# unirestore/UniRestore

Hardware: AMD Instinct MI355X
Metric: restored 512x512 images/sec @ 20 denoise steps (whole job) (higher is better)
Workload: dtype bf16; 1 GPU; PIR 512x512 batch=8/GPU, 20 DDIM steps, bf16, hipGraph replay (BASELINE.json configs[1]; configs[2] shape for N=8); global_batch=8, per_gpu_batch=8, image=512, denoise_steps=20, parallelism=image-parallel dp1, weights=seeded random init (no checkpoints reachable)

## Files before the change

### include/unirestore_hip.h

```cpp
#ifndef UNIRESTORE_HIP_H
#define UNIRESTORE_HIP_H

#include <stddef.h>
#include <stdint.h>

#ifdef __cplusplus
extern "C" {
#endif

typedef void* ur_stream_t;

enum { UR_OK = 0, UR_E_INVALID = -1, UR_E_UNSUPPORTED = -2, UR_E_LAUNCH = -3, UR_E_WORKSPACE = -4 };

enum { UR_DT_BF16 = 0, UR_DT_F16 = 1 };

enum {
  UR_ACT_NONE = 0,
  UR_ACT_SILU = 1,
  UR_ACT_GELU = 2,
  UR_ACT_GEGLU = 3,
  UR_ACT_GATE = 4,
  UR_ACT_TANH = 5,
  UR_ACT_RELU = 6
};
// ... 60 lines not shown
int ur_conv2d_plan_launch(const ur_conv_desc* d, ur_conv_launch_info* info);
int ur_conv_launcher_count(void);
const char* ur_conv_launcher_name(int i);

int ur_gemm_bias_act(const void* x, const void* w, const float* bias, const void* residual, void* y, long long M, int N, int K,
                     int ldx, int ldw, int ldy, int ldr, int act, float* workspace, size_t workspace_bytes, int dtype,
                     ur_stream_t stream);
int ur_groupconv3x3_nhwc(const void* x, const void* w, const float* bias, void* y, int N, int H, int W, int Cg, int Cog,
                         int groups, int act, float* workspace, size_t workspace_bytes, int dtype, ur_stream_t stream);

int ur_groupnorm_stats_parts(int N, int HW, int C);
size_t ur_groupnorm_ws_bytes(int N, int HW, int C);
size_t ur_groupnorm_ab_bytes(int N, int C);
int ur_groupnorm_stats(const void* x, float* part, int N, int HW, int C, int dtype, ur_stream_t stream);
int ur_instnorm_stats(const void* x, float* part, int N, int HW, int C, int dtype, ur_stream_t stream);
int ur_groupnorm_finalize(const float* part1, int parts1, int C1, const float* part2, int parts2, int C2, const float* gamma,
                          const float* beta, int N, int HW, int G, float eps, float* ab, float* mean_out, ur_stream_t stream);
int ur_groupnorm_apply_act(const void* x, const void* x2, void* y, const float* ab, int N, int HW, int C1, int C2, int silu,
                           int dtype, ur_stream_t stream);
int ur_groupnorm_nhwc(const void* x, const void* x2, void* y, const float* gamma, const float* beta, int N, int HW,
                      int C1, int C2, int G, float eps, int silu, float* ws, float* ab, const float* pre1, int parts1,
                      const float* pre2, int parts2, int dtype, ur_stream_t stream);
int ur_layernorm_rows(const void* x, void* y, const float* gamma, const float* beta, long long rows, int C,
                      float eps, int dtype, ur_stream_t stream);
int ur_softmax_rows_f32(const float* s, void* p, long long rows, int cols, int ldp, int dtype, ur_stream_t stream);

int ur_attention_fwd(const void* q, const void* k, const void* vt, void* o, int B, int H, int Tq, int Tk,
                     int D, int ldq, int ldk, int ldvt, int ldo, long long bs_q, long long bs_k,
                     long long bs_vt, long long bs_o, float scale, int dtype, ur_stream_t stream);
size_t ur_attention_workspace_bytes(int B, int H, int Tq, int Tk, int D);
// ... 81 lines not shown
```

### unirestore_amd/capi.py

```python
import ctypes as C
import os

import torch

_HERE = os.path.dirname(os.path.abspath(__file__))
LIB_PATH = os.environ.get("UR_LIB") or os.path.join(_HERE, "libunirestore_hip.so")

UR_ACT_NONE, UR_ACT_SILU, UR_ACT_GELU, UR_ACT_GEGLU, UR_ACT_GATE, UR_ACT_TANH, UR_ACT_RELU = range(7)
UR_DT_BF16, UR_DT_F16 = 0, 1
UR_E_INVALID, UR_E_UNSUPPORTED = -1, -2


class ConvDesc(C.Structure):
    _fields_ = [
        ("x", C.c_void_p), ("x2", C.c_void_p), ("w", C.c_void_p), ("bias", C.c_void_p), ("residual", C.c_void_p),
        ("y", C.c_void_p), ("yt", C.c_void_p), ("gn_part", C.c_void_p), ("gn_ab", C.c_void_p), ("gn_silu", C.c_int),
        ("row_stats", C.c_void_p), ("ln_stats", C.c_void_p), ("ln_colsum", C.c_void_p), ("ln_eps", C.c_float), ("ln_dim", C.c_int), ("ln_parts", C.c_int),
        ("workspace", C.c_void_p),
        ("workspace_bytes", C.c_size_t),
        ("N", C.c_int), ("H", C.c_int), ("W", C.c_int),
        ("C1", C.c_int), ("ldx", C.c_int), ("C2", C.c_int), ("ldx2", C.c_int),
        ("Cout", C.c_int), ("ldw", C.c_int), ("ldy", C.c_int), ("ldr", C.c_int),
        ("KH", C.c_int), ("KW", C.c_int), ("stride", C.c_int), ("pad_t", C.c_int), ("pad_l", C.c_int),
        ("OH", C.c_int), ("OW", C.c_int),
# ... 25 lines not shown
SIGNATURES = {
    "ur_version": (_I, []),
    "ur_last_error": (C.c_char_p, []),
    "ur_conv2d_nhwc": (_I, [C.POINTER(ConvDesc), _P]),
    "ur_conv2d_plan": (_I, [C.POINTER(ConvDesc), C.POINTER(ConvPlan)]),
    "ur_conv2d_plan_launch": (_I, [C.POINTER(ConvDesc), C.POINTER(ConvLaunchInfo)]),
    "ur_conv_launcher_count": (_I, []),
    "ur_conv_launcher_name": (C.c_char_p, [_I]),
    "ur_gemm_bias_act": (_I, [_P, _P, _P, _P, _P, _LL, _I, _I, _I, _I, _I, _I, _I, _P, _SZ, _I, _P]),
    "ur_groupconv3x3_nhwc": (_I, [_P, _P, _P, _P, _I, _I, _I, _I, _I, _I, _I, _P, _SZ, _I, _P]),
    "ur_groupnorm_stats_parts": (_I, [_I, _I, _I]),
    "ur_groupnorm_ws_bytes": (_SZ, [_I, _I, _I]),
    "ur_groupnorm_ab_bytes": (_SZ, [_I, _I]),
    "ur_groupnorm_stats": (_I, [_P, _P, _I, _I, _I, _I, _P]),
    "ur_instnorm_stats": (_I, [_P, _P, _I, _I, _I, _I, _P]),
    "ur_groupnorm_finalize": (_I, [_P, _I, _I, _P, _I, _I, _P, _P, _I, _I, _I, _F, _P, _P, _P]),
    "ur_groupnorm_apply_act": (_I, [_P, _P, _P, _P, _I, _I, _I, _I, _I, _I, _P]),
    "ur_groupnorm_nhwc": (_I, [_P, _P, _P, _P, _P, _I, _I, _I, _I, _I, _F, _I, _P, _P, _P, _I, _P, _I, _I, _P]),
    "ur_layernorm_rows": (_I, [_P, _P, _P, _P, _LL, _I, _F, _I, _P]),
    "ur_softmax_rows_f32": (_I, [_P, _P, _LL, _I, _I, _I, _P]),
    "ur_attention_fwd": (_I, [_P, _P, _P, _P, _I, _I, _I, _I, _I, _I, _I, _I, _I, _LL, _LL, _LL, _LL, _F, _I, _P]),
    "ur_attention_workspace_bytes": (_SZ, [_I, _I, _I, _I, _I]),
    "ur_attention_fwd_ws": (_I, [_P, _P, _P, _P, _I, _I, _I, _I, _I, _I, _I, _I, _I, _LL, _LL, _LL, _LL, _F, _P, _SZ, _I, _P]),
    "ur_attention_plan_launch": (_I, [_P, _P, _P, _P, _I, _I, _I, _I, _I, _I, _I, _I, _I, _LL, _LL, _LL, _LL, _P, _SZ, C.POINTER(AttentionPlan)]),
    "ur_attention_kernel_count": (_I, []),
    "ur_attention_kernel_name": (C.c_char_p, [_I]),
    "ur_chain_tile_bytes": (_SZ, []),
    "ur_ff_geglu_fused": (_I, [_P, _P, _SZ, _P, _LL, _I, _I, _I, _I, _F, _I, _P]),
    "ur_transformer_head_fused": (_I, [_P, _P, _P, _SZ, _P, _P, _P, _P, _LL, _I, _I, _F, _I, _P]),
    "ur_transformer_tail_fused": (_I, [_P, _P, _P, _P, _SZ, _P, _P, _LL, _I, _I, _I, _I, _I, _F, _F, _I, _P]),
# ... 79 lines not shown
```

### unirestore_amd/csrc/igemm.hip

```cpp
#include "igemm_impl.h"

namespace urk {
#define UR_DECLARE(name)                                                                                             \
  ConvLaunch name##_bf16(void* k, size_t ws_bytes);                                                                 \
  ConvLaunch name##_f16(void* k, size_t ws_bytes);                                                                  \
  static ConvLaunch name(ConvK& k, size_t ws_bytes) { return (k.f16 ? name##_f16 : name##_bf16)(&k, ws_bytes); }
UR_CONV_LAUNCHERS(UR_DECLARE)
#undef UR_DECLARE
}

namespace {

ConvLaunch dispatch_conv(ConvK& k, bool pair, size_t ws_bytes) {
  if (k.KH == 3 && k.stride == 1 && k.pad_t == 1 && k.pad_l == 1 && k.kcm && k.staged_ok_ && !pair && k.nbatch == 1 &&
      k.OW % 32 == 0 && k.OH % 8 == 0 && k.OH == (k.ups ? 2 * k.H : k.H) && k.OW == (k.ups ? 2 * k.W : k.W) && !k.yt) {
    const bool ok128 = k.Cout % 128 == 0, ok160 = k.Cout % 160 == 0;
    const long long tm8 = (long long)k.N * (k.OH / 8) * (k.OW / 32);
    auto eff = [](long long t) { return t <= 128 ? (double)(t * (256 / t)) / 256.0 : (double)t / (double)(((t + 255) / 256) * 256); };
    const bool use160 = ok160 && (!ok128 || eff(tm8 * (k.Cout / 160)) >= eff(tm8 * (k.Cout / 128)));
    const long long tiles8 = tm8 * (use160 ? k.Cout / 160 : k.Cout / 128);
    if ((ok128 || ok160) && tiles8 >= 64) {
      if (use160) return urk::halo_8x32_160(k, ws_bytes);
      return urk::halo_8x32_128(k, ws_bytes);
    }
// ... 12 lines not shown
    if (k.OH == 8 && k.OW == 8 && k.N % 4 == 0) {
      return urk::himg_8x8x4(k, ws_bytes);
    }
  }
  if (k.KH == 1 && k.stride == 1 && !k.ups && k.C2 == 0 && k.staged_ok_ && k.Cout % 256 == 0 && !k.yt && (k.act == UR_ACT_GEGLU || k.act == UR_ACT_GATE) &&
      (long long)((k.M + 255) / 256) * (k.Cout / 256) * k.nbatch >= 200 && (long long)k.M * k.ldx < (1ll << 31) - 256)
  {
    auto fill = [](long long t) { return (double)t / (double)(((t + 255) / 256) * 256); };
    const long long tm = (k.M + 255) / 256;
    if (k.Cout % 320 == 0 && k.nbatch == 1 && !k.bias_img && fill(tm * (k.Cout / 320)) > fill(tm * (k.Cout / 256)))
      return urk::gemm_256x320_pair(k, ws_bytes);
    return urk::gemm_256x256(k, ws_bytes);
  }
  const bool use_v1 = k.KH == 1 && k.nk <= 10;
  const long long blocks128 = (long long)((k.M + 127) / 128) * ((k.Cout + 127) / 128) * k.nbatch;
  const bool g1 = k.KH == 1 && k.stride == 1 && !k.ups && k.C2 == 0 && k.pad_t == 0 && k.pad_l == 0 && k.OH == k.H && k.OW == k.W &&
                  (long long)k.M * k.ldx + k.Ktot < (1ll << 31) - 256;
  auto nosplit = [&](int bm, int bn) { return (long long)((k.M + bm - 1) / bm) * ((k.Cout + bn - 1) / bn) * k.nbatch >= 200 || k.nk < 8 || !k.ws; };
  if (k.KH == 1 && !pair && k.Cout > 64) {
    const long long blocks64 = (long long)((k.M + 63) / 64) * ((k.Cout + 63) / 64) * k.nbatch;
    if (blocks128 < 200 && g1 && blocks64 >= 128 && blocks64 <= 256 && k.nk >= 8 && k.nk <= 48) return urk::g1_64x64_deep(k, ws_bytes);
    if (g1 && blocks128 < 200 && k.nk > 24 && k.nk <= 96 && (long long)((k.M + 127) / 128) * ((k.Cout + 63) / 64) * k.nbatch >= 256)
      return urk::g1_128x64_deep(k, ws_bytes);
    if (blocks128 < 200 && g1 && ((blocks64 >= 128 && k.nk <= 24) || (blocks64 >= 256 && k.nk <= 48))) return urk::g1_64x64(k, ws_bytes);
    if (blocks128 < 200 && k.nk <= 24) return g1 && nosplit(64, 64) ? urk::g1_64x64(k, ws_bytes) : urk::v1_64x64(k, ws_bytes);
    if (use_v1 && blocks128 > 256 && blocks128 < 400 && k.Cout % 128 == 0) return g1 && nosplit(128, 64) ? urk::g1_128x64(k, ws_bytes) : urk::v1_128x64(k, ws_bytes);
  }
  if (use_v1) {
    if (pair) return urk::v1_128x128(k, ws_bytes);
    if (k.Cout <= 32) return urk::v1_256x32(k, ws_bytes);
    if (k.Cout <= 64) return urk::v1_128x64(k, ws_bytes);
// ... 177 lines not shown
```

### unirestore_amd/csrc/igemm_g1.hip

```cpp
#include "igemm_impl.h"

#ifndef UR_NST_128x128
#define UR_NST_128x128 2
#endif
#ifndef UR_NST_128x160
#define UR_NST_128x160 2
#endif
#ifndef UR_NST_128x64
#define UR_NST_128x64 2
#endif
#ifndef UR_NST_64x64
#define UR_NST_64x64 2
#endif

namespace urk {
UR_LAUNCHER(g1_128x128, Gemm<128, 128, 2, 2, UR_NST_128x128, true>)
UR_LAUNCHER(g1_128x160, Gemm<128, 160, 4, 1, UR_NST_128x160, true>)
UR_LAUNCHER(g1_128x64, Gemm<128, 64, 2, 2, UR_NST_128x64, true>)
UR_LAUNCHER(g1_64x64, Gemm<64, 64, 2, 2, UR_NST_64x64, true>)
UR_LAUNCHER(g1_64x64_deep, Gemm<64, 64, 2, 2, 4, true>)
UR_LAUNCHER(g1_128x64_deep, Gemm<128, 64, 2, 2, 3, true>)
}
```

### unirestore_amd/csrc/igemm_impl.h

```cpp
#pragma once
#include <cstdio>
#include <cstdlib>
#include <map>
#include <string>

#include "common.h"

static __device__ uint4 g_zero_page[8];
typedef uint32_t ig_u32x4 __attribute__((ext_vector_type(4)));

struct ConvLaunch {
  int (*launch)(void* k, hipStream_t s);
  int prologue_ok;
  int id;
};

namespace {

struct ConvK {
  const uint16_t* x; const uint16_t* x2; const uint16_t* w; const float* bias; const uint16_t* res;
  void* y; uint16_t* yt; float* ws; float* gn_part; const float* gn_ab;
  float* row_stats; const float* ln_stats; const float* ln_colsum; float ln_eps; int ln_dim, ln_parts;
  int N, H, W, C1, ldx, C2, ldx2, Cin, Cout, ldw, ldy, ldr, KH, KW, stride, pad_t, pad_l, OH, OW, OHW;
  int ups, act, out_f32, n_split, t_rows, t_ld;
// ... 1050 lines not shown
__device__ __forceinline__ ig_u32x4 ig_make_rsrc(const void* base, unsigned long long bytes) {
  const unsigned long long a = (unsigned long long)base;
  ig_u32x4 r;
  r[0] = __builtin_amdgcn_readfirstlane((unsigned)a);
  r[1] = __builtin_amdgcn_readfirstlane((unsigned)(a >> 32) & 0xffffu);
  r[2] = __builtin_amdgcn_readfirstlane((unsigned)(bytes < IG_OOB ? bytes : IG_OOB));
  r[3] = 0x00020000u;
  return r;
}
__device__ __forceinline__ void ig_lds_dma16(unsigned m0v, unsigned voff, const ig_u32x4& rs, unsigned soff) {
  asm volatile("s_mov_b32 m0, %0\n\ts_nop 0\n\tbuffer_load_dwordx4 %1, %2, %3 offen lds" ::"s"(__builtin_amdgcn_readfirstlane(m0v)), "v"(voff), "s"(rs),
               "s"(__builtin_amdgcn_readfirstlane(soff)) : "memory");
}


template <int BM, int BN, int WM, int WN, int NST, bool DIRECT, bool PAIRC, bool F16>
__global__ __launch_bounds__(WM* WN * 64) void gemm_glds_kernel(const ConvK p) {
  constexpr int NT = WM * WN * 64, RPP = NT / 8;
  constexpr int WTM = BM / WM, WTN = BN / WN, FM = WTM / 32, FN = WTN / 32;
  constexpr int XP = BM / RPP, WP = BN / RPP, NLD = XP + WP;
  constexpr int STAGE = (BM + BN) * 128;
  static_assert(BM % RPP == 0 && BN % RPP == 0 && WTM % 32 == 0 && WTN % 32 == 0 && RPP % 16 == 0, "tile/wave shape");
  extern __shared__ __attribute__((aligned(16))) unsigned char smem[];
  const int tid = threadIdx.x, lane = tid & 63, wid = tid >> 6;
  const int wm = wid % WM, wn = wid / WM;
  const int gb = blockIdx.y;
  int tm, tn;
  xcd_tile_map(p, blockIdx.x, tm, tn);
  const int m0 = tm * BM, n0 = tn * BN;
  const uint16_t* __restrict__ X1 = p.x + gb * p.bs_x;
  const uint16_t* __restrict__ Wt = p.w + gb * p.bs_w;
  const uint16_t* zero = reinterpret_cast<const uint16_t*>(g_zero_page);
// ... 22 lines not shown
      const uint16_t* g = (kval && woff[j] >= 0) ? Wt + woff[j] + kbase : zero;
      __builtin_amdgcn_global_load_lds((gptr_t)g, (lptr_t)(wsm + (j * RPP + wid * 8) * 128), 16, 0, 0);
    }
    kbase += 64;
  };
#else
  const ig_u32x4 rs_x = ig_make_rsrc(X1, (unsigned long long)p.M * p.ldx * 2);
  const ig_u32x4 rs_w = ig_make_rsrc(Wt, (unsigned long long)p.Cout * p.ldw * 2);
  const unsigned smem_lds = (unsigned)(uintptr_t)(lptr_t)smem;
  const int wid_s = __builtin_amdgcn_readfirstlane(wid);
  unsigned xvo[XP], wvo[WP];
#pragma unroll
  for (int i = 0; i < XP; ++i) { const int m = m0 + i * RPP + lrow; xvo[i] = m < p.M ? ((unsigned)m * (unsigned)p.ldx + chunk * 8u) * 2u : IG_OOB; }
#pragma unroll
  for (int j = 0; j < WP; ++j) { const int r = n0 + j * RPP + lrow; wvo[j] = r < p.Cout ? ((unsigned)r * (unsigned)p.ldw + chunk * 8u) * 2u : IG_OOB; }
  auto issue_tile = [&](int stage) {
    const unsigned xs = smem_lds + stage * STAGE, wsm = xs + BM * 128;
    const bool kval = kbase + chunk * 8 < p.Ktot;
    const unsigned so = (unsigned)kbase * 2u;
#pragma unroll
    for (int i = 0; i < XP; ++i) ig_lds_dma16(xs + (i * RPP + wid_s * 8) * 128, kval ? xvo[i] : IG_OOB, rs_x, so);
#pragma unroll
    for (int j = 0; j < WP; ++j) ig_lds_dma16(wsm + (j * RPP + wid_s * 8) * 128, kval ? wvo[j] : IG_OOB, rs_w, so);
    kbase += 64;
  };
#endif
  f32x16 acc[FN][FM];
#pragma unroll
  for (int a = 0; a < FN; ++a)
#pragma unroll
    for (int b = 0; b < FM; ++b)
#pragma unroll
      for (int e = 0; e < 16; ++e) acc[a][b][e] = 0.f;
  const int frow = lane & 31, fhalf = lane >> 5;
// ... 36 lines not shown
#pragma unroll
      for (int a = 0; a < FN; ++a)
#pragma unroll
        for (int b = 0; b < FM; ++b)
          acc[a][b] = mfma16t(afr[a], bfr[b], acc[a][b]);
    }
    cs = (cs + 1 == NST) ? 0 : cs + 1;
    if (NST >= 3 && issued - (t + 1) >= NST - 1) asm volatile("s_waitcnt vmcnt(%0) lgkmcnt(0)" ::"n"(NLD * (NST >= 3 ? NST - 2 : 0)) : "memory");
    else asm volatile("s_waitcnt vmcnt(0) lgkmcnt(0)" ::: "memory");
    __builtin_amdgcn_s_barrier();
  }
  if constexpr (ktile_gemm_ok<FM, FN>()) asm volatile("s_nop 15\n\ts_nop 7" ::: "memory");
  igemm_epilogue<FM, FN, WTM, WTN, BM, BN, NT, F16, DIRECT, PAIRC>(p, acc, m0, n0, wm, wn, lane, gb, 0, smem);
}

template <int BM, int BN, int WM, int WN, int NST, bool DIRECT = false, bool PAIRC = false>
struct Gemm {
  static constexpr int lds_loop = NST * (BM + BN) * 128, lds_epi = epi_lds_bytes<BM, BN, WM * WN * 64, PAIRC>();
  static constexpr int lds = lds_loop > lds_epi ? lds_loop : lds_epi;
  static_assert(lds <= 160 * 1024, "LDS budget");
  static int plan(ConvK& k, size_t) {
    k.tiles_m = (k.M + BM - 1) / BM;
    k.tiles_n = (k.Cout + BN - 1) / BN;
    k.splitk = 1;
    k.nk_per_split = k.nk;
    set_gn_plan(k, k.staged_ok_ && (k.OHW % BM) == 0, k.OHW / BM);
    return 0;
  }
  static int launch(ConvK& k, hipStream_t s) {
    static ur::DeviceOnce attr_once;
    if (auto once_guard = attr_once.first()) {
      hipFuncSetAttribute(reinterpret_cast<const void*>(&gemm_glds_kernel<BM, BN, WM, WN, NST, DIRECT, PAIRC, UR_TU_F16 != 0>), hipFuncAttributeMaxDynamicSharedMemorySize, lds);
    }
    pick_xcd_grid(k, (double)k.Cout * k.Ktot, (double)k.M * k.Cin);
    UR_F16_SWITCH(k, hipLaunchKernelGGL((gemm_glds_kernel<BM, BN, WM, WN, NST, DIRECT, PAIRC, F16>), dim3(k.tiles_m * k.tiles_n, k.nbatch, 1), dim3(WM * WN * 64), lds, s, k));
    return ur::check_launch("ur_conv2d_nhwc");
  }
};

template <int BM, int BN, int WM, int WN, int NST, int MIN_BLOCKS>
struct Glds {
  static constexpr int lds_loop = NST * (BM + BN) * 128, lds_epi = epi_lds_bytes<BM, BN, WM * WN * 64>();
  static constexpr int lds = lds_loop > lds_epi ? lds_loop : lds_epi;
  static int plan(ConvK& k, size_t ws_bytes) {
    k.tiles_m = (k.M + BM - 1) / BM;
    k.tiles_n = (k.Cout + BN - 1) / BN;
    const long long blocks = (long long)k.tiles_m * k.tiles_n * k.nbatch;
    long long want = 1;
    if (blocks < MIN_BLOCKS && k.nk >= 8 && k.ws && k.y && !k.row_stats && !k.ln_stats)
// ... 989 lines not shown
```

### unirestore_amd/csrc/norms.hip

```cpp
#include <cstdio>
#include <cstdlib>
#include <map>
#include <string>
#include "common.h"

namespace {

template <bool F16>
__global__ __launch_bounds__(256) void gn_stats_kernel(const uint16_t* __restrict__ x, float* __restrict__ part,
                                                       int HW, int C, int pix_per_block, int CVS) {
  __shared__ float lds[256 * 16];
  const int n = blockIdx.y, t = threadIdx.x, P = gridDim.x;
  const int CV = C >> 3, R = 256 / CVS;
  const int r = t / CVS, vl = t - r * CVS, v = blockIdx.z * CVS + vl;
  const int p_begin = blockIdx.x * pix_per_block, p_end = min(HW, p_begin + pix_per_block);
  float s[8] = {0, 0, 0, 0, 0, 0, 0, 0}, q[8] = {0, 0, 0, 0, 0, 0, 0, 0};
  if (r < R && v < CV) {
    const uint16_t* xi = x + (long long)n * HW * C + v * 8;
    for (int p = p_begin + r; p < p_end; p += 4 * R) {
      uint4 raw[4];
#pragma unroll
      for (int u = 0; u < 4; ++u) {
        const int pp = min(p + u * R, p_end - 1);
        raw[u] = *reinterpret_cast<const uint4*>(xi + (long long)pp * C);
// ... 7 lines not shown
        for (int e = 0; e < 8; ++e) { s[e] += f[e]; q[e] += f[e] * f[e]; }
      }
    }
  }
  if (r < R) {
#pragma unroll
    for (int e = 0; e < 8; ++e) { lds[(r * 2) * CVS * 8 + vl * 8 + e] = s[e]; lds[(r * 2 + 1) * CVS * 8 + vl * 8 + e] = q[e]; }
  }
  __syncthreads();
  for (int i = t; i < CVS * 8; i += 256) {
    const int c = blockIdx.z * CVS * 8 + i;
    if (c >= C) continue;
    float a = 0.f, b = 0.f;
    for (int rr = 0; rr < R; ++rr) { a += lds[(rr * 2) * CVS * 8 + i]; b += lds[(rr * 2 + 1) * CVS * 8 + i]; }
    *reinterpret_cast<float2*>(part + (((long long)n * P + blockIdx.x) * C + c) * 2) = make_float2(a, b);
  }
}

__global__ void gn_finalize_kernel(const float* __restrict__ p1, int P1, int C1, const float* __restrict__ p2, int P2, int C2,
                                   const float* __restrict__ gamma, const float* __restrict__ beta, int G, float eps,
                                   double inv_cnt, float* __restrict__ ab, float* __restrict__ mean_out) {
  __shared__ double red[2][256];
  const int g = blockIdx.x, n = blockIdx.y, t = threadIdx.x, NT = blockDim.x;
  const int C = C1 + C2, cpg = C / G, c_lo = g * cpg, Pmax = max(P1, P2);
  float ga0 = 1.f, be0 = 0.f;
  if (ab && t < cpg) { ga0 = gamma ? gamma[c_lo + t] : 1.f; be0 = beta ? beta[c_lo + t] : 0.f; }
  double s = 0.0, q = 0.0;
  for (int idx = t; idx < cpg * Pmax; idx += NT) {
    const int p = idx / cpg, c = c_lo + (idx - p * cpg);
    const bool first = c < C1;
// ... 175 lines not shown

}

static void gn_geom(int N, int HW, int C, int ppt, int& cvs, int& slabs, int& chunks, int& ppb) {
  const int cv = C / 8;
  cvs = cv < 32 ? cv : 32;
  while (cv % cvs) --cvs;
  slabs = cv / cvs;
  const int R = 256 / cvs;
  const long long want = std::max<long long>(1, 2048 / ((long long)N * slabs));
  chunks = (int)std::min<long long>(want, std::max(1, HW / ((HW <= 64 ? std::min(ppt, 2) : ppt) * R)));
  ppb = (HW + chunks - 1) / chunks;
  chunks = (HW + ppb - 1) / ppb;
}

namespace ur {
int gn_stats_parts(int N, int HW, int C) {
  int cvs, slabs, chunks, ppb;
  gn_geom(N, HW, C, 8, cvs, slabs, chunks, ppb);
  return chunks;
}
int gn_stats_launch(const void* x, float* part, int N, int HW, int C, int dtype, hipStream_t s) {
  int cvs, slabs, chunks, ppb;
  gn_geom(N, HW, C, 8, cvs, slabs, chunks, ppb);
  UR_DT_SWITCH(dtype, hipLaunchKernelGGL(gn_stats_kernel<F16>, dim3(chunks, N, slabs), dim3(256), 0, s, (const uint16_t*)x, part, HW, C, ppb, cvs));
  return check_launch("gn_stats");
}
}

extern "C" {

int ur_groupnorm_stats_parts(int N, int HW, int C) { return (N > 0 && HW > 0 && C > 0 && C % 8 == 0) ? ur::gn_stats_parts(N, HW, C) : UR_E_INVALID; }
size_t ur_groupnorm_ws_bytes(int N, int HW, int C) { return (size_t)N * (size_t)std::max(ur_groupnorm_stats_parts(N, HW, C), 1) * C * 2 * sizeof(float); }
size_t ur_groupnorm_ab_bytes(int N, int C) { return (size_t)N * C * 2 * sizeof(float); }

int ur_groupnorm_stats(const void* x, float* part, int N, int HW, int C, int dtype, ur_stream_t stream) {
  UR_REQUIRE(x && part && N > 0 && HW > 0 && C > 0 && C % 8 == 0, "bad args");
  UR_REQUIRE_DT(dtype);
  hipStream_t s = (hipStream_t)stream;
  ur::ProfScope prof("groupnorm_stats", 0.0, 2.0 * N * HW * (double)C, s);
  return ur::gn_stats_launch(x, part, N, HW, C, dtype, s);
}
int ur_instnorm_stats(const void* x, float* part, int N, int HW, int C, int dtype, ur_stream_t stream) {
  return ur_groupnorm_stats(x, part, N, HW, C, dtype, stream);
}

int ur_groupnorm_finalize(const float* part1, int parts1, int C1, const float* part2, int parts2, int C2, const float* gamma,
                          const float* beta, int N, int HW, int G, float eps, float* ab, float* mean_out, ur_stream_t stream) {
  const int C = C1 + (part2 ? C2 : 0);
  UR_REQUIRE(part1 && parts1 > 0 && C1 > 0 && (!part2 || (parts2 > 0 && C2 > 0)), "bad partial planes");
  UR_REQUIRE(G > 0 && C % G == 0 && N > 0 && HW > 0 && (ab || mean_out), "bad args");
  hipStream_t s = (hipStream_t)stream;
  const int cpg = C / G;
  const long long entries = (long long)cpg * std::max(parts1, part2 ? parts2 : 0);
  ur::ProfScope prof("groupnorm_finalize", 0.0, 8.0 * N * ((double)parts1 * C1 + (part2 ? (double)parts2 * C2 : 0.0)), s);
  const int nt = entries <= 1024 ? 64 : 256;
  hipLaunchKernelGGL(gn_finalize_kernel, dim3(G, N), dim3(nt), 0, s, part1, parts1, C1, part2, part2 ? parts2 : 0, part2 ? C2 : 0, gamma, beta, G,
                     eps, 1.0 / ((double)cpg * HW), ab, mean_out);
  return ur::check_launch("ur_groupnorm_finalize");
// ... 106 lines not shown
```

### unirestore_amd/modules/model.py

```python
import os
import weakref
from typing import Optional

import numpy as np
import torch
import torch.nn as nn
import torch.nn.functional as F

from .. import ops, schedule, tiling
from .adapters import SPADE, CSCEAdapter, TaskFeatureAdapter, cfrm_blocks
from . import nn as nnmod
from .nn import (DEV, AutoencoderKL, Conv2d, DownBlock, MidBlock, ResnetBlock2D, TimestepEmbedding, UNet2DConditionModel,
                 invalidate_packed, sinusoid_table)

stablesr_config = dict(in_channels=4, model_channels=256, out_channels=256, num_res_blocks=2, dropout=0,
                       channel_mult=(1, 1, 2, 2), downsample_type="conv", num_heads=4,
                       down_block_types=("AttnDownBlock2D",) * 3 + ("DownBlock2D",), mid_block_type="UNetMidBlock2D")


TILE_CONTROLLER_MAX_IMAGES = 400


def _use_dtype(module):
    owner = module.__dict__.get("_ur_owner")
# ... 49 lines not shown
        for m in self.modules():
            if isinstance(m, ResnetBlock2D):
                nn.init.zeros_(m.conv2.weight), nn.init.zeros_(m.conv2.bias)
            if hasattr(m, "to_out") and hasattr(m, "group_norm"):
                nn.init.zeros_(m.to_out[0].weight), nn.init.zeros_(m.to_out[0].bias)

    def set_timesteps(self, timesteps):
        emb = self.time_embedding.silu_emb(sinusoid_table(timesteps, self.model_channels))
        for r in _resnets(self):
            r.set_time_table(emb)
        self.table_epoch = getattr(self, "table_epoch", 0) + 1

    def stem(self, z_bf16):
        return ops.conv(z_bf16, self.conv_in.packed(), gn=True)

    def run(self, stem, step):
        feats, h = [], stem
        for blk in self.down_blocks:
            states = []
            for i, res in enumerate(blk.resnets):
                h = res.run(h, step=step)
                if blk.attn_kind == "self":
                    h = blk.attentions[i].run(h)
                states.append(h)
            if blk.downsamplers is not None:
                h = blk.downsamplers[0].run(h)
                states.append(h)
            feats.append(states[-2])
        feats[-1] = self.middle_block.run(h, step=step)
        return {f.shape[2]: self.fea_tran[i].run(f, step=step) for i, f in enumerate(feats)}

    def run_schedule(self, stem, nsteps):
        b = stem.shape[0]
        x = stem.repeat(nsteps, 1, 1, 1)
        g = ops.gn_of(stem)
        if g is not None:
            x._gn = (g[0].repeat(nsteps, 1, 1, 1), g[1])
        out = self.run(x, "all")
        return [{k: v[i * b:(i + 1) * b] for k, v in out.items()} for i in range(nsteps)]

    def run_steps(self, stem, s0, s1):
        b, n = stem.shape[0], s1 - s0
        x = stem.repeat(n, 1, 1, 1)
        g = ops.gn_of(stem)
        if g is not None:
            x._gn = (g[0].repeat(n, 1, 1, 1), g[1])
        out = self.run(x, slice(s0, s1))
        return [{k: v[i * b:(i + 1) * b] for k, v in out.items()} for i in range(n)]

    def forward(self, x, timesteps, encoder_hidden_states=None):
        _use_dtype(self)
        ts = _per_sample_timesteps(timesteps, x.shape[0])
        self.set_timesteps(ts)
        out = self.run(self.stem(ops.nchw_to_nhwc(x.to(DEV))), 0 if len(ts) == 1 else "all")
        out = {k: ops.nhwc_to_nchw(v) for k, v in out.items()}
        _check_fp16(out)
        return out


class ControlledUNet(nn.Module):
    def __init__(self, unet: UNet2DConditionModel, control_type: str, null_embeds: Optional[torch.Tensor] = None,
                 cond_channels: int = 256):
# ... 614 lines not shown
```

### unirestore_amd/modules/nn.py

```python
import math
from typing import Optional

import os

import torch
import torch.nn as nn

from .. import chain, ops
from ..ops import UR_ACT_GEGLU, UR_ACT_GELU, UR_ACT_NONE, UR_ACT_SILU

DEV = "cuda"
CHAIN = os.environ.get("UR_CHAIN", "1") == "1"


class _NoEager:
    def forward(self, *a, **k):
        raise RuntimeError(f"{type(self).__name__}: no eager/PyTorch path exists; use the HIP-backed graph")


class Conv2d(_NoEager, nn.Conv2d):
    def packed(self, pair=False, scale: Optional[torch.Tensor] = None) -> ops.PackedConv:
        key = ("pk", pair, ops.act_dtype())
        if key not in self.__dict__:
            w, b = self.weight, self.bias
# ... 106 lines not shown
                bias = self._tbias_all(x.shape[0] // (step.stop - step.start), step)
            else:
                bias = self.tbias[step]
        h = gn_silu_conv(self.norm1, x, self.conv1.packed(), x2=x2, bias=bias, gn=True)
        pc2 = self.conv2.packed()
        if self.conv_shortcut is not None:
            sc = ops.conv(x, self.conv_shortcut.packed(), x2=x2)
        else:
            sc = x
        if control is not None and "spade" in self._modules:
            if x2 is not None and self.conv_shortcut is None:
                raise ValueError("identity shortcut cannot take a virtual concat")
            h = gn_silu_conv(self.norm2, h, pc2, gn=True)
            return self.spade.run(h, control[h.shape[2]], residual=sc)
        return gn_silu_conv(self.norm2, h, pc2, residual=sc, gn=True)


FUSE_GN_MIN_PIXELS = 256 * 256
FUSE_GN_MAX_COUT = 256


def gn_silu_conv(norm: "GroupNorm", x, pc, x2=None, **kw):
    ab = norm.coeffs(x, x2=x2)
    if x.shape[1] * x.shape[2] >= FUSE_GN_MIN_PIXELS and pc.cout_out <= FUSE_GN_MAX_COUT and \
            ops.conv_plan(x, pc, x2=x2, gn=kw.get("gn", False), gn_ab=True, residual=kw.get("residual") is not None).prologue_ok:
        return ops.conv(x, pc, x2=x2, gn_ab=ab, gn_silu=True, **kw)
    return ops.conv(ops.gn_apply(x, ab, silu=True, x2=x2), pc, **kw)


class Downsample2D(nn.Module):
# ... 376 lines not shown
```

### unirestore_amd/ops.py

```python
from dataclasses import dataclass
from typing import Optional

import torch

from . import capi
from .capi import (UR_ACT_GATE, UR_ACT_GEGLU, UR_ACT_GELU, UR_ACT_NONE, UR_ACT_RELU, UR_ACT_SILU, UR_ACT_TANH, UR_DT_BF16,
                   UR_DT_F16, ConvDesc, ConvPlan, check, lib)

BF16 = torch.bfloat16
F16 = torch.float16
_ws = {}

_DTYPES = {"bf16": BF16, "bfloat16": BF16, BF16: BF16, "fp16": F16, "float16": F16, "f16": F16, "16": F16, F16: F16}
_act = BF16


def set_dtype(dt) -> torch.dtype:
    global _act
    if dt not in _DTYPES:
        raise ValueError(f"unsupported compute dtype {dt!r}: choose 'bf16' or 'fp16'")
    _act = _DTYPES[dt]
    return _act


# ... 147 lines not shown
         out_hw=None, upsample=False, out_f32=False, out_scale=1.0, out=None, yt=None, n_split=0, t_rows=0,
         gn=False, store=True, rows=False, ln_stats=None, gn_ab=None, gn_silu=False):
    if x.dtype not in (BF16, F16) or x.dtype != pc.w.dtype or not x.is_contiguous() or x.dim() != 4:
        raise ValueError(f"conv: x must be a contiguous 4-d {pc.w.dtype} tensor, got {x.dtype} {tuple(x.shape)}")
    n, h, w_, c1 = x.shape
    c2 = 0 if x2 is None else x2.shape[-1]
    if (c1 + c2) != pc.cin * pc.groups:
        raise ValueError(f"conv: Cin mismatch: {c1}+{c2} vs {pc.cin}*{pc.groups}")
    d = _conv_desc(x, pc, x2, stride, pad, upsample, out_hw, plan_only=False)
    assert not pc.kcm or d.k_chunk_major, "chunk-major weights need a 64-aligned concat boundary"
    oh, ow = d.OH, d.OW
    co_total = pc.cout_out
    if out is None and store:
        out = torch.empty((n, oh, ow, co_total), dtype=torch.float32 if out_f32 else x.dtype, device=x.device)
    bias_t = pc.bias if bias is None else bias
    d.bias = _ptr(bias_t)
    if bias is not None and bias.dim() == 2 and bias.shape[0] > 1:
        d.bias_img_stride = bias.shape[1]
    d.residual, d.y, d.yt = _ptr(residual), _ptr(out), _ptr(yt)
    if ln_stats is not None:
        assert pc.ln_colsum is not None, "weights were not packed with pack_linear_ln"
        st, parts = ln_stats
        d.ln_stats, d.ln_colsum, d.ln_eps, d.ln_dim, d.ln_parts = st.data_ptr(), pc.ln_colsum.data_ptr(), pc.ln_eps, pc.cin, parts
    if gn_ab is not None:
        d.gn_ab, d.gn_silu = gn_ab.data_ptr(), int(gn_silu)
    if out is not None:
        d.ldy = out.shape[-1]
    d.ldr = residual.shape[-1] if residual is not None else 0
    d.act, d.out_f32, d.out_scale = act, int(out_f32), out_scale
    d.n_split, d.t_rows = n_split, t_rows
# ... 116 lines not shown
def gn_finalize(x: torch.Tensor, gamma, beta, groups: int, eps: float, x2=None, use_pre=True, want_mean=False):
    n, c1 = x.shape[0], x.shape[-1]
    c2 = 0 if x2 is None else x2.shape[-1]
    hw = x.numel() // (n * c1)
    if not use_pre:
        x = x.view(x.shape)
        x2 = None if x2 is None else x2.view(x2.shape)
    p1, n1 = gn_partials(x)
    p2, n2 = gn_partials(x2) if x2 is not None else (None, 0)
    out = torch.empty((n, groups) if want_mean else (n, 2, c1 + c2), dtype=torch.float32, device=x.device)
    check(lib.ur_groupnorm_finalize(p1.data_ptr(), n1, c1, _ptr(p2), n2, c2, _ptr(gamma), _ptr(beta), n, hw, groups, eps,
                                    None if want_mean else out.data_ptr(), out.data_ptr() if want_mean else None, _stream()))
    return out


def gn_finalize_planes(plane: torch.Tensor, parts: int, hw: int):
    n, c = plane.shape[0], plane.shape[2]
    out = torch.empty((n, c), dtype=torch.float32, device=plane.device)
    check(lib.ur_groupnorm_finalize(plane.data_ptr(), parts, c, None, 0, 0, None, None, n, hw, c, 0.0, None, out.data_ptr(), _stream()))
    return out


def gn_apply(x: torch.Tensor, ab: torch.Tensor, silu=False, x2=None):
    n, c1 = x.shape[0], x.shape[-1]
    c2 = 0 if x2 is None else x2.shape[-1]
    hw = x.numel() // (n * c1)
    out = torch.empty((*x.shape[:-1], c1 + c2), dtype=x.dtype, device=x.device)
    check(lib.ur_groupnorm_apply_act(x.data_ptr(), _ptr(x2), out.data_ptr(), ab.data_ptr(), n, hw, c1, c2, int(silu), _dt(x), _stream()))
    return out

# ... 293 lines not shown
```

Before: 31.04 images/s.

## Run first control resnet conv once and expand per-step time bias with fused GN stats

The control encoder's first resnet used to process the stem repeated once per denoise step. Its first conv input is identical across steps, so it now runs once without bias into fp32. A new kernel then expands the result across steps by adding each step's time-embedding bias, writing bf16 and emitting groupnorm partial stats in the same pass. Separately, the 1x1 pure-GEMM kernels gain a two-source variant that reads concatenated inputs directly, so more convs take the g1 path. This adds an fp32 intermediate and only applies when there is an identity shortcut and no SPADE; otherwise run_stacked raises.

```diff
diff --git a/include/unirestore_hip.h b/include/unirestore_hip.h
--- a/include/unirestore_hip.h
+++ b/include/unirestore_hip.h
@@ -98,6 +98,9 @@
 size_t ur_groupnorm_ab_bytes(int N, int C);
 int ur_groupnorm_stats(const void* x, float* part, int N, int HW, int C, int dtype, ur_stream_t stream);
 int ur_instnorm_stats(const void* x, float* part, int N, int HW, int C, int dtype, ur_stream_t stream);
+int ur_bias_expand_parts(int HW, int C);
+int ur_bias_expand_gn(const float* acc, const float* bias, void* y, float* gn_part, int B, int S, int HW, int C, int dtype,
+                      ur_stream_t stream);
 int ur_groupnorm_finalize(const float* part1, int parts1, int C1, const float* part2, int parts2, int C2, const float* gamma,
                           const float* beta, int N, int HW, int G, float eps, float* ab, float* mean_out, ur_stream_t stream);
 int ur_groupnorm_apply_act(const void* x, const void* x2, void* y, const float* ab, int N, int HW, int C1, int C2, int silu,
diff --git a/unirestore_amd/capi.py b/unirestore_amd/capi.py
--- a/unirestore_amd/capi.py
+++ b/unirestore_amd/capi.py
@@ -63,6 +63,8 @@
     "ur_groupnorm_ab_bytes": (_SZ, [_I, _I]),
     "ur_groupnorm_stats": (_I, [_P, _P, _I, _I, _I, _I, _P]),
     "ur_instnorm_stats": (_I, [_P, _P, _I, _I, _I, _I, _P]),
+    "ur_bias_expand_parts": (_I, [_I, _I]),
+    "ur_bias_expand_gn": (_I, [_P, _P, _P, _P, _I, _I, _I, _I, _I, _P]),
     "ur_groupnorm_finalize": (_I, [_P, _I, _I, _P, _I, _I, _P, _P, _I, _I, _I, _F, _P, _P, _P]),
     "ur_groupnorm_apply_act": (_I, [_P, _P, _P, _P, _I, _I, _I, _I, _I, _I, _P]),
     "ur_groupnorm_nhwc": (_I, [_P, _P, _P, _P, _P, _I, _I, _I, _I, _I, _F, _I, _P, _P, _P, _I, _P, _I, _I, _P]),
diff --git a/unirestore_amd/csrc/igemm.hip b/unirestore_amd/csrc/igemm.hip
--- a/unirestore_amd/csrc/igemm.hip
+++ b/unirestore_amd/csrc/igemm.hip
@@ -50,7 +50,8 @@
   }
   const bool use_v1 = k.KH == 1 && k.nk <= 10;
   const long long blocks128 = (long long)((k.M + 127) / 128) * ((k.Cout + 127) / 128) * k.nbatch;
-  const bool g1 = k.KH == 1 && k.stride == 1 && !k.ups && k.C2 == 0 && k.pad_t == 0 && k.pad_l == 0 && k.OH == k.H && k.OW == k.W &&
+  const bool two_src = k.C2 == 0 || (k.C1 % 64 == 0 && k.C2 % 8 == 0 && !use_v1 && (long long)k.M * k.ldx2 + k.C2 < (1ll << 31) - 256);
+  const bool g1 = k.KH == 1 && k.stride == 1 && !k.ups && two_src && k.pad_t == 0 && k.pad_l == 0 && k.OH == k.H && k.OW == k.W &&
                   (long long)k.M * k.ldx + k.Ktot < (1ll << 31) - 256;
   auto nosplit = [&](int bm, int bn) { return (long long)((k.M + bm - 1) / bm) * ((k.Cout + bn - 1) / bn) * k.nbatch >= 200 || k.nk < 8 || !k.ws; };
   if (k.KH == 1 && !pair && k.Cout > 64) {
diff --git a/unirestore_amd/csrc/igemm_g1.hip b/unirestore_amd/csrc/igemm_g1.hip
--- a/unirestore_amd/csrc/igemm_g1.hip
+++ b/unirestore_amd/csrc/igemm_g1.hip
@@ -14,10 +14,10 @@
 #endif
 
 namespace urk {
-UR_LAUNCHER(g1_128x128, Gemm<128, 128, 2, 2, UR_NST_128x128, true>)
-UR_LAUNCHER(g1_128x160, Gemm<128, 160, 4, 1, UR_NST_128x160, true>)
+UR_LAUNCHER(g1_128x128, Gemm<128, 128, 2, 2, UR_NST_128x128, true, false, true>)
+UR_LAUNCHER(g1_128x160, Gemm<128, 160, 4, 1, UR_NST_128x160, true, false, true>)
 UR_LAUNCHER(g1_128x64, Gemm<128, 64, 2, 2, UR_NST_128x64, true>)
-UR_LAUNCHER(g1_64x64, Gemm<64, 64, 2, 2, UR_NST_64x64, true>)
-UR_LAUNCHER(g1_64x64_deep, Gemm<64, 64, 2, 2, 4, true>)
-UR_LAUNCHER(g1_128x64_deep, Gemm<128, 64, 2, 2, 3, true>)
+UR_LAUNCHER(g1_64x64, Gemm<64, 64, 2, 2, UR_NST_64x64, true, false, true>)
+UR_LAUNCHER(g1_64x64_deep, Gemm<64, 64, 2, 2, 4, true, false, true>)
+UR_LAUNCHER(g1_128x64_deep, Gemm<128, 64, 2, 2, 3, true, false, true>)
 }
diff --git a/unirestore_amd/csrc/igemm_impl.h b/unirestore_amd/csrc/igemm_impl.h
--- a/unirestore_amd/csrc/igemm_impl.h
+++ b/unirestore_amd/csrc/igemm_impl.h
@@ -1088,8 +1088,8 @@
 }
 
 
-template <int BM, int BN, int WM, int WN, int NST, bool DIRECT, bool PAIRC, bool F16>
-__global__ __launch_bounds__(WM* WN * 64) void gemm_glds_kernel(const ConvK p) {
+template <int BM, int BN, int WM, int WN, int NST, bool DIRECT, bool PAIRC, bool F16, bool TWO>
+__device__ __forceinline__ void gemm_glds_body(const ConvK& p) {
   constexpr int NT = WM * WN * 64, RPP = NT / 8;
   constexpr int WTM = BM / WM, WTN = BN / WN, FM = WTM / 32, FN = WTN / 32;
   constexpr int XP = BM / RPP, WP = BN / RPP, NLD = XP + WP;
@@ -1142,10 +1142,26 @@
   for (int i = 0; i < XP; ++i) { const int m = m0 + i * RPP + lrow; xvo[i] = m < p.M ? ((unsigned)m * (unsigned)p.ldx + chunk * 8u) * 2u : IG_OOB; }
 #pragma unroll
   for (int j = 0; j < WP; ++j) { const int r = n0 + j * RPP + lrow; wvo[j] = r < p.Cout ? ((unsigned)r * (unsigned)p.ldw + chunk * 8u) * 2u : IG_OOB; }
+  const ig_u32x4 rs_x2 = TWO ? ig_make_rsrc(p.x2 + gb * p.bs_x2, (unsigned long long)p.M * p.ldx2 * 2) : rs_x;
+  unsigned xvo2[TWO ? XP : 1];
+  if constexpr (TWO) {
+#pragma unroll
+    for (int i = 0; i < XP; ++i) { const int m = m0 + i * RPP + lrow; xvo2[i] = m < p.M ? ((unsigned)m * (unsigned)p.ldx2 + chunk * 8u) * 2u : IG_OOB; }
+  }
   auto issue_tile = [&](int stage) {
     const unsigned xs = smem_lds + stage * STAGE, wsm = xs + BM * 128;
     const bool kval = kbase + chunk * 8 < p.Ktot;
     const unsigned so = (unsigned)kbase * 2u;
+    if constexpr (TWO) {
+      if (kbase >= p.C1) {
+        const unsigned so2 = (unsigned)(kbase - p.C1) * 2u;
+#pragma unroll
+        for (int i = 0; i < XP; ++i) ig_lds_dma16(xs + (i * RPP + wid_s * 8) * 128, kval ? xvo2[i] : IG_OOB, rs_x2, so2);
+      } else {
+#pragma unroll
+        for (int i = 0; i < XP; ++i) ig_lds_dma16(xs + (i * RPP + wid_s * 8) * 128, kval ? xvo[i] : IG_OOB, rs_x, so);
+      }
+    } else
 #pragma unroll
     for (int i = 0; i < XP; ++i) ig_lds_dma16(xs + (i * RPP + wid_s * 8) * 128, kval ? xvo[i] : IG_OOB, rs_x, so);
 #pragma unroll
@@ -1212,7 +1228,16 @@
   igemm_epilogue<FM, FN, WTM, WTN, BM, BN, NT, F16, DIRECT, PAIRC>(p, acc, m0, n0, wm, wn, lane, gb, 0, smem);
 }
 
-template <int BM, int BN, int WM, int WN, int NST, bool DIRECT = false, bool PAIRC = false>
+template <int BM, int BN, int WM, int WN, int NST, bool DIRECT, bool PAIRC, bool F16>
+__global__ __launch_bounds__(WM* WN * 64) void gemm_glds_kernel(const ConvK p) {
+  gemm_glds_body<BM, BN, WM, WN, NST, DIRECT, PAIRC, F16, false>(p);
+}
+template <int BM, int BN, int WM, int WN, int NST, bool DIRECT, bool PAIRC, bool F16>
+__global__ __launch_bounds__(WM* WN * 64) void gemm_glds2_kernel(const ConvK p) {
+  gemm_glds_body<BM, BN, WM, WN, NST, DIRECT, PAIRC, F16, true>(p);
+}
+
+template <int BM, int BN, int WM, int WN, int NST, bool DIRECT = false, bool PAIRC = false, bool TWOSRC = false>
 struct Gemm {
   static constexpr int lds_loop = NST * (BM + BN) * 128, lds_epi = epi_lds_bytes<BM, BN, WM * WN * 64, PAIRC>();
   static constexpr int lds = lds_loop > lds_epi ? lds_loop : lds_epi;
@@ -1231,6 +1256,17 @@
       hipFuncSetAttribute(reinterpret_cast<const void*>(&gemm_glds_kernel<BM, BN, WM, WN, NST, DIRECT, PAIRC, UR_TU_F16 != 0>), hipFuncAttributeMaxDynamicSharedMemorySize, lds);
     }
     pick_xcd_grid(k, (double)k.Cout * k.Ktot, (double)k.M * k.Cin);
+    if (k.C2 != 0) {
+      if constexpr (TWOSRC) {
+        static ur::DeviceOnce attr2_once;
+        if (auto once_guard = attr2_once.first()) {
+          hipFuncSetAttribute(reinterpret_cast<const void*>(&gemm_glds2_kernel<BM, BN, WM, WN, NST, DIRECT, PAIRC, UR_TU_F16 != 0>), hipFuncAttributeMaxDynamicSharedMemorySize, lds);
+        }
+        UR_F16_SWITCH(k, hipLaunchKernelGGL((gemm_glds2_kernel<BM, BN, WM, WN, NST, DIRECT, PAIRC, F16>), dim3(k.tiles_m * k.tiles_n, k.nbatch, 1), dim3(WM * WN * 64), lds, s, k));
+        return ur::check_launch("ur_conv2d_nhwc");
+      }
+      return ur::fail(UR_E_UNSUPPORTED, "ur_conv2d_nhwc: this pure-GEMM launcher has no two-source kernel");
+    }
     UR_F16_SWITCH(k, hipLaunchKernelGGL((gemm_glds_kernel<BM, BN, WM, WN, NST, DIRECT, PAIRC, F16>), dim3(k.tiles_m * k.tiles_n, k.nbatch, 1), dim3(WM * WN * 64), lds, s, k));
     return ur::check_launch("ur_conv2d_nhwc");
   }
diff --git a/unirestore_amd/csrc/norms.hip b/unirestore_amd/csrc/norms.hip
--- a/unirestore_amd/csrc/norms.hip
+++ b/unirestore_amd/csrc/norms.hip
@@ -45,6 +45,66 @@
     float a = 0.f, b = 0.f;
     for (int rr = 0; rr < R; ++rr) { a += lds[(rr * 2) * CVS * 8 + i]; b += lds[(rr * 2 + 1) * CVS * 8 + i]; }
     *reinterpret_cast<float2*>(part + (((long long)n * P + blockIdx.x) * C + c) * 2) = make_float2(a, b);
+  }
+}
+
+constexpr int EXP_U = 8;
+template <bool F16>
+__global__ __launch_bounds__(256) void bias_expand_gn_kernel(const float* __restrict__ acc, const float* __restrict__ bias,
+                                                             uint16_t* __restrict__ y, float* __restrict__ part, int B, int S,
+                                                             int HW, int C, int pix_per_block, int CVS) {
+  __shared__ float lds[256 * 16];
+  const int i = blockIdx.y, t = threadIdx.x, P = gridDim.x;
+  const int CV = C >> 3, R = 256 / CVS;
+  const int r = t / CVS, vl = t - r * CVS, v = blockIdx.z * CVS + vl;
+  const int p_begin = blockIdx.x * pix_per_block, p_end = min(HW, p_begin + pix_per_block);
+  const bool active = r < R && v < CV;
+  float a[EXP_U][8];
+  if (active) {
+    const float* ai = acc + (long long)i * HW * C + v * 8;
+#pragma unroll
+    for (int u = 0; u < EXP_U; ++u) {
+      const int pp = min(p_begin + r + u * R, p_end - 1);
+      const float4 lo = *reinterpret_cast<const float4*>(ai + (long long)pp * C);
+      const float4 hi = *reinterpret_cast<const float4*>(ai + (long long)pp * C + 4);
+      a[u][0] = lo.x; a[u][1] = lo.y; a[u][2] = lo.z; a[u][3] = lo.w; a[u][4] = hi.x; a[u][5] = hi.y; a[u][6] = hi.z; a[u][7] = hi.w;
+    }
+  }
+  for (int st = 0; st < S; ++st) {
+    const int n = st * B + i;
+    float s[8] = {0, 0, 0, 0, 0, 0, 0, 0}, q[8] = {0, 0, 0, 0, 0, 0, 0, 0};
+    if (active) {
+      float b[8];
+#pragma unroll
+      for (int e = 0; e < 8; ++e) b[e] = bias[(long long)st * C + v * 8 + e];
+      uint16_t* yo = y + (long long)n * HW * C + v * 8;
+#pragma unroll
+      for (int u = 0; u < EXP_U; ++u) {
+        const int pp = p_begin + r + u * R;
+        if (pp >= p_end) break;
+        float f[8];
+#pragma unroll
+        for (int e = 0; e < 8; ++e) f[e] = a[u][e] + b[e];
+        const uint4 o = pack8t<F16>(f);
+        store16_wt(yo + (long long)pp * C, o);
+        unpack8t<F16>(o, f);
+#pragma unroll
+        for (int e = 0; e < 8; ++e) { s[e] += f[e]; q[e] += f[e] * f[e]; }
+      }
+    }
+    if (r < R) {
+#pragma unroll
+      for (int e = 0; e < 8; ++e) { lds[(r * 2) * CVS * 8 + vl * 8 + e] = s[e]; lds[(r * 2 + 1) * CVS * 8 + vl * 8 + e] = q[e]; }
+    }
+    __syncthreads();
+    for (int j = t; j < CVS * 8; j += 256) {
+      const int c = blockIdx.z * CVS * 8 + j;
+      if (c >= C) continue;
+      float sa = 0.f, sb = 0.f;
+      for (int rr = 0; rr < R; ++rr) { sa += lds[(rr * 2) * CVS * 8 + j]; sb += lds[(rr * 2 + 1) * CVS * 8 + j]; }
+      *reinterpret_cast<float2*>(part + (((long long)n * P + blockIdx.x) * C + c) * 2) = make_float2(sa, sb);
+    }
+    __syncthreads();
   }
 }
 
@@ -250,6 +310,13 @@
   chunks = (HW + ppb - 1) / ppb;
 }
 
+static void expand_geom(int HW, int C, int& cvs, int& slabs, int& chunks, int& ppb) {
+  int unused_chunks, unused_ppb;
+  gn_geom(1, HW, C, 8, cvs, slabs, unused_chunks, unused_ppb);
+  ppb = std::min(HW, EXP_U * (256 / cvs));
+  chunks = (HW + ppb - 1) / ppb;
+}
+
 namespace ur {
 int gn_stats_parts(int N, int HW, int C) {
   int cvs, slabs, chunks, ppb;
@@ -279,6 +346,26 @@
 }
 int ur_instnorm_stats(const void* x, float* part, int N, int HW, int C, int dtype, ur_stream_t stream) {
   return ur_groupnorm_stats(x, part, N, HW, C, dtype, stream);
+}
+
+int ur_bias_expand_parts(int HW, int C) {
+  if (HW <= 0 || C <= 0 || C % 8 != 0) return UR_E_INVALID;
+  int cvs, slabs, chunks, ppb;
+  expand_geom(HW, C, cvs, slabs, chunks, ppb);
+  return chunks;
+}
+int ur_bias_expand_gn(const float* acc, const float* bias, void* y, float* gn_part, int B, int S, int HW, int C, int dtype,
+                      ur_stream_t stream) {
+  UR_REQUIRE(acc && bias && y && gn_part && B > 0 && S > 0 && HW > 0 && C > 0 && C % 8 == 0, "bad args");
+  UR_REQUIRE(B <= 65535 && (long long)S * B * HW * C < (1ll << 40), "batch too large");
+  UR_REQUIRE_DT(dtype);
+  hipStream_t s = (hipStream_t)stream;
+  ur::ProfScope prof("bias_expand_gn", 0.0, (double)B * HW * C * (4.0 + 2.0 * S), s);
+  int cvs, slabs, chunks, ppb;
+  expand_geom(HW, C, cvs, slabs, chunks, ppb);
+  UR_DT_SWITCH(dtype, hipLaunchKernelGGL(bias_expand_gn_kernel<F16>, dim3(chunks, B, slabs), dim3(256), 0, s, acc, bias, (uint16_t*)y, gn_part, B, S,
+                                         HW, C, ppb, cvs));
+  return ur::check_launch("ur_bias_expand_gn");
 }
 
 int ur_groupnorm_finalize(const float* part1, int parts1, int C1, const float* part2, int parts2, int C2, const float* gamma,
diff --git a/unirestore_amd/modules/model.py b/unirestore_amd/modules/model.py
--- a/unirestore_amd/modules/model.py
+++ b/unirestore_amd/modules/model.py
@@ -87,12 +87,12 @@
     def stem(self, z_bf16):
         return ops.conv(z_bf16, self.conv_in.packed(), gn=True)
 
-    def run(self, stem, step):
+    def run(self, stem, step, stack=1):
         feats, h = [], stem
-        for blk in self.down_blocks:
+        for bi, blk in enumerate(self.down_blocks):
             states = []
             for i, res in enumerate(blk.resnets):
-                h = res.run(h, step=step)
+                h = res.run_stacked(h, step, stack) if stack > 1 and bi == 0 and i == 0 else res.run(h, step=step)
                 if blk.attn_kind == "self":
                     h = blk.attentions[i].run(h)
                 states.append(h)
@@ -104,21 +104,21 @@
         return {f.shape[2]: self.fea_tran[i].run(f, step=step) for i, f in enumerate(feats)}
 
     def run_schedule(self, stem, nsteps):
+        return self._run_stacked(stem, "all", nsteps)
+
+    def run_steps(self, stem, s0, s1):
+        return self._run_stacked(stem, slice(s0, s1), s1 - s0)
+
+    def _run_stacked(self, stem, step, n):
         b = stem.shape[0]
-        x = stem.repeat(nsteps, 1, 1, 1)
-        g = ops.gn_of(stem)
-        if g is not None:
-            x._gn = (g[0].repeat(nsteps, 1, 1, 1), g[1])
-        out = self.run(x, "all")
-        return [{k: v[i * b:(i + 1) * b] for k, v in out.items()} for i in range(nsteps)]
-
-    def run_steps(self, stem, s0, s1):
-        b, n = stem.shape[0], s1 - s0
-        x = stem.repeat(n, 1, 1, 1)
-        g = ops.gn_of(stem)
-        if g is not None:
-            x._gn = (g[0].repeat(n, 1, 1, 1), g[1])
-        out = self.run(x, slice(s0, s1))
+        if n > 1:
+            out = self.run(stem, step, stack=n)
+        else:
+            x = stem.repeat(n, 1, 1, 1)
+            g = ops.gn_of(stem)
+            if g is not None:
+                x._gn = (g[0].repeat(n, 1, 1, 1), g[1])
+            out = self.run(x, step)
         return [{k: v[i * b:(i + 1) * b] for k, v in out.items()} for i in range(n)]
 
     def forward(self, x, timesteps, encoder_hidden_states=None):
diff --git a/unirestore_amd/modules/nn.py b/unirestore_amd/modules/nn.py
--- a/unirestore_amd/modules/nn.py
+++ b/unirestore_amd/modules/nn.py
@@ -144,6 +144,14 @@
             h = gn_silu_conv(self.norm2, h, pc2, gn=True)
             return self.spade.run(h, control[h.shape[2]], residual=sc)
         return gn_silu_conv(self.norm2, h, pc2, residual=sc, gn=True)
+
+    def run_stacked(self, x, step, nsteps):
+        rows = self.tbias if isinstance(step, str) else self.tbias[step]
+        if rows.shape[0] != nsteps or self.conv_shortcut is not None or "spade" in self._modules:
+            raise ValueError("run_stacked: one bias row per stacked step, identity shortcut, no SPADE")
+        acc = gn_silu_conv(self.norm1, x, self.conv1.packed(), bias=False, out_f32=True)
+        h = ops.bias_expand_gn(acc, rows, x.dtype)
+        return gn_silu_conv(self.norm2, h, self.conv2.packed(), residual=x.repeat(nsteps, 1, 1, 1), gn=True)
 
 
 FUSE_GN_MIN_PIXELS = 256 * 256
diff --git a/unirestore_amd/ops.py b/unirestore_amd/ops.py
--- a/unirestore_amd/ops.py
+++ b/unirestore_amd/ops.py
@@ -185,6 +185,8 @@
     if out is None and store:
         out = torch.empty((n, oh, ow, co_total), dtype=torch.float32 if out_f32 else x.dtype, device=x.device)
     bias_t = pc.bias if bias is None else bias
+    if bias is False:
+        bias_t = bias = None
     d.bias = _ptr(bias_t)
     if bias is not None and bias.dim() == 2 and bias.shape[0] > 1:
         d.bias_img_stride = bias.shape[1]
@@ -331,6 +333,23 @@
     return out
 
 
+def bias_expand_gn(acc: torch.Tensor, bias: torch.Tensor, dtype=None):
+    b, h, w_, c = acc.shape
+    s = bias.shape[0]
+    if acc.dtype != torch.float32 or bias.dtype != torch.float32 or not acc.is_contiguous() or not bias.is_contiguous() or bias.shape[1] != c:
+        raise ValueError(f"bias_expand_gn: contiguous fp32 acc [B,H,W,C] and bias [S,C] wanted, got {tuple(acc.shape)} {tuple(bias.shape)}")
+    dtype = dtype or _act
+    parts = lib.ur_bias_expand_parts(h * w_, c)
+    if parts <= 0:
+        check(parts if parts < 0 else -1)
+    out = torch.empty((s * b, h, w_, c), dtype=dtype, device=acc.device)
+    plane = torch.empty((s * b, parts, c, 2), dtype=torch.float32, device=acc.device)
+    check(lib.ur_bias_expand_gn(acc.data_ptr(), bias.data_ptr(), out.data_ptr(), plane.data_ptr(), b, s, h * w_, c,
+                                UR_DT_F16 if dtype == F16 else UR_DT_BF16, _stream()))
+    out._gn = (plane, parts)
+    return out
+
+
 def gn_finalize_planes(plane: torch.Tensor, parts: int, hw: int):
     n, c = plane.shape[0], plane.shape[2]
     out = torch.empty((n, c), dtype=torch.float32, device=plane.device)
```

New measurement: 31.33 images/s (median of 6 runs). About the same (+0.9%).
